# fr34za/multilinear

Measured on NVIDIA B200. Metric: pcs_commit_melem_per_s, higher is better.
Workload: dtype u128

## Files before the change

include/multilinear_b200_instr.h:

```cpp
#ifndef MULTILINEAR_B200_INSTR_H
#define MULTILINEAR_B200_INSTR_H
#include <stddef.h>
#include <stdint.h>

#ifdef __cplusplus
extern "C" {
#endif

void ml_trace_dump(void);

int ml_profile_enable(int on);
int ml_profile_reset(void);
int ml_profile_get(int id, double *total_ms, uint64_t *launches, double *alg_bytes);
int ml_profile_get_max(int id, double *mean_ms, uint64_t *launches, double *alg_bytes);
int ml_microbench(const char *what, size_t n, int iters, double *ms_out, double *work_out);

struct ml_shard;
int ml_shard_phase_ms(const struct ml_shard *sh, double *out, int cap);
struct ml_pcs_shard;
int ml_pcs_shard_phase_ms(const struct ml_pcs_shard *sh, double *out, int cap);
struct ml_bpcs_shard;
int ml_bpcs_shard_phase_ms(const struct ml_bpcs_shard *sh, double *out, int cap);

#ifdef __cplusplus
}
#endif
#endif
```

multilinear_b200/api.py:

```python
import ctypes as C

import numpy as np

from ._lib import MlError, NotPowerOfTwo, NotRsCode, SizeMismatch, check, load

M = 340282366920938463463374557953744961537
LOG_BLOWUP = 1
NUM_QUERIES = 128
_sz = C.c_size_t


def _p(a):
    return C.c_void_p(a.ctypes.data)


def aligned_empty(nbytes, align=64):
    raw = np.empty(nbytes + align, dtype=np.uint8)
    off = (-raw.ctypes.data) % align
    return raw[off:off + nbytes]


def elems_empty(n):
    return aligned_empty(16 * n).reshape(n, 16)

# ... 1028 lines not shown
    def free(self):
        if self.h is not None and self.h.value:
            load().ml_wsumcheck_shard_free(self.h)
        self.h = None

    def __del__(self):
        try:
            self.free()
        except Exception:
            pass


_INSTR = None


def microbench(what, n, iters):
    global _INSTR
    if _INSTR is None:
        import os
        load()
        _INSTR = C.CDLL(os.path.join(os.path.dirname(os.path.abspath(__file__)), "libmlb_instr.so"))
    ms, work = C.c_double(0), C.c_double(0)
    check(_INSTR.ml_microbench(what.encode(), _sz(n), C.c_int(iters), C.byref(ms), C.byref(work)))
    return ms.value, work.value
```

multilinear_b200/csrc/field.cuh:

```cuda
#pragma once
#include <cstdint>
#include <cuda_runtime.h>

namespace mlb {

struct fe {
    uint32_t v[4];
};

#define MLB_C0 0xFFFFFFFFu
#define MLB_C1 0x00002CFFu
#define MLB_M0 0x00000001u
#define MLB_M1 0xFFFFD300u
#define MLB_M2 0xFFFFFFFFu
#define MLB_M3 0xFFFFFFFFu

__device__ __forceinline__ fe fe_zero() { return fe{{0u, 0u, 0u, 0u}}; }
__device__ __forceinline__ fe fe_one() { return fe{{1u, 0u, 0u, 0u}}; }
__device__ __forceinline__ fe fe_from_u4(uint4 x) { return fe{{x.x, x.y, x.z, x.w}}; }
__device__ __forceinline__ uint4 fe_to_u4(fe a) { return make_uint4(a.v[0], a.v[1], a.v[2], a.v[3]); }
__device__ __forceinline__ fe fe_load(const fe* p) { return fe_from_u4(*reinterpret_cast<const uint4*>(p)); }
__device__ __forceinline__ fe fe_load_nc(const fe* p) { return fe_from_u4(__ldg(reinterpret_cast<const uint4*>(p))); }
__device__ __forceinline__ void fe_store(fe* p, fe a) { *reinterpret_cast<uint4*>(p) = fe_to_u4(a); }
__device__ __forceinline__ bool fe_eq(fe a, fe b) {
// ... 83 lines not shown
    uint32_t y0 = x0, y1 = x1, y2 = x2, y3 = x3, k1, q0, q1, q2, k2;
    asm("mad.lo.cc.u32 %0, %5, %7, %0; madc.hi.cc.u32 %1, %5, %7, %1; madc.lo.cc.u32 %2, %6, %8, %2; madc.hi.cc.u32 %3, %6, %8, %3; addc.u32 %4, 0, 0;"
        : "+r"(y0), "+r"(y1), "+r"(y2), "+r"(y3), "=&r"(k1) : "r"(x4), "r"(x5), "r"(c0), "r"(c1));
    asm("mul.lo.u32 %0, %3, %5; mul.hi.u32 %1, %3, %5; mad.lo.cc.u32 %0, %4, %6, %0; madc.hi.cc.u32 %1, %4, %6, %1; addc.u32 %2, 0, 0;"
        : "=&r"(q0), "=&r"(q1), "=&r"(q2) : "r"(x4), "r"(x5), "r"(c1), "r"(c0));
    asm("add.cc.u32 %0, %0, %4; addc.cc.u32 %1, %1, %5; addc.cc.u32 %2, %2, %6; addc.u32 %3, 0, 0;"
        : "+r"(y1), "+r"(y2), "+r"(y3), "=&r"(k2) : "r"(q0), "r"(q1), "r"(q2));
    uint32_t m = 0u - (k1 + k2);
    asm("add.cc.u32 %0, %0, %4; addc.cc.u32 %1, %1, %5; addc.cc.u32 %2, %2, 0; addc.u32 %3, %3, 0;"
        : "+r"(y0), "+r"(y1), "+r"(y2), "+r"(y3) : "r"(m & c0), "r"(m & c1));
    return fe_new(fe{{y0, y1, y2, y3}});
}


#define MLB_K45 11520u
__device__ __forceinline__ fe fe_reduce_wide_v2(const uint32_t p[8]) {
    uint32_t a1 = p[1], a2 = p[2], a3 = p[3], a4, a5, x0, x1, x2, x3, x4, x5;
    const uint32_t k = MLB_K45;
    asm("mad.lo.cc.u32 %0, %4, %6, %0; madc.hi.cc.u32 %1, %4, %6, %1; madc.lo.cc.u32 %2, %5, %6, %2; madc.hi.u32 %3, %5, %6, 0;"
        : "+r"(a1), "+r"(a2), "+r"(a3), "=&r"(a4) : "r"(p[4]), "r"(p[6]), "r"(k));
    asm("mad.lo.cc.u32 %0, %4, %6, %0; madc.hi.cc.u32 %1, %4, %6, %1; madc.lo.cc.u32 %2, %5, %6, %2; madc.hi.u32 %3, %5, %6, 0;"
        : "+r"(a2), "+r"(a3), "+r"(a4), "=&r"(a5) : "r"(p[5]), "r"(p[7]), "r"(k));
    asm("sub.cc.u32 %0, %6, %12; subc.cc.u32 %1, %7, %13; subc.cc.u32 %2, %8, %14; subc.cc.u32 %3, %9, %15; subc.cc.u32 %4, %10, 0; subc.u32 %5, %11, 0;"
        : "=&r"(x0), "=&r"(x1), "=&r"(x2), "=&r"(x3), "=&r"(x4), "=&r"(x5)
        : "r"(p[0]), "r"(a1), "r"(a2), "r"(a3), "r"(a4), "r"(a5), "r"(p[4]), "r"(p[5]), "r"(p[6]), "r"(p[7]));
    const unsigned long long U = (unsigned long long)x4 * MLB_K45 + ((unsigned long long)(x5 * MLB_K45) << 32);
    uint32_t b1, b2, b3, k1, y0, y1, y2, y3, k2;
    asm("add.cc.u32 %0, %4, %7; addc.cc.u32 %1, %5, %8; addc.cc.u32 %2, %6, 0; addc.u32 %3, 0, 0;"
        : "=&r"(b1), "=&r"(b2), "=&r"(b3), "=&r"(k1) : "r"(x1), "r"(x2), "r"(x3), "r"((uint32_t)U), "r"((uint32_t)(U >> 32)));
    asm("sub.cc.u32 %0, %5, %9; subc.cc.u32 %1, %6, %10; subc.cc.u32 %2, %7, 0; subc.cc.u32 %3, %8, 0; subc.u32 %4, 0, 0;"
        : "=&r"(y0), "=&r"(y1), "=&r"(y2), "=&r"(y3), "=&r"(k2) : "r"(x0), "r"(b1), "r"(b2), "r"(b3), "r"(x4), "r"(x5));
    uint32_t z0, z1, z2, z3, g;
    asm("add.cc.u32 %0, %5, %9; addc.cc.u32 %1, %6, %10; addc.cc.u32 %2, %7, 0; addc.cc.u32 %3, %8, 0; addc.u32 %4, %11, %12;"
        : "=&r"(z0), "=&r"(z1), "=&r"(z2), "=&r"(z3), "=&r"(g)
        : "r"(y0), "r"(y1), "r"(y2), "r"(y3), "r"(MLB_C0), "r"(MLB_C1), "r"(k1), "r"(k2));
    return fe{{g ? z0 : y0, g ? z1 : y1, g ? z2 : y2, g ? z3 : y3}};
}
#ifndef MLB_REDUCE_V
#define MLB_REDUCE_V 2
#endif
template <int V>
__device__ __forceinline__ fe fe_reduce_wide_t(const uint32_t p[8]) { return V == 1 ? fe_reduce_wide_v1(p) : fe_reduce_wide_v2(p); }
__device__ __forceinline__ fe fe_reduce_wide(const uint32_t p[8]) { return fe_reduce_wide_t<MLB_REDUCE_V>(p); }
template <int V>
__device__ __forceinline__ fe fe_mul_t(const fe& a, const fe& b) {
    uint32_t p[8];
    fe_mul_wide(p, a, b);
    return fe_reduce_wide_t<V>(p);
}

__device__ __forceinline__ fe fe_mul(const fe& a, const fe& b) {
    uint32_t p[8];
    fe_mul_wide(p, a, b);
    return fe_reduce_wide(p);
}
__device__ __forceinline__ fe fe_sqr(const fe& a) { return fe_mul(a, a); }

__device__ inline fe fe_pow_u64(fe base, unsigned long long e) {
    fe r = fe_one();
    while (e) {
        if (e & 1ull) r = fe_mul(r, base);
        base = fe_sqr(base);
        e >>= 1;
    }
    return r;
}

struct fe_acc {
    uint32_t w[9];
};
__device__ __forceinline__ void acc_zero(fe_acc& s) {
#pragma unroll
// ... 23 lines not shown
```

multilinear_b200/csrc/internal.h:

```cpp
#pragma once
#include <atomic>
#include <cstdarg>
#include <cstdint>
#include <cstdio>
#include <cstring>
#include <map>
#include <mutex>
#include <vector>

#include <cuda_runtime.h>

#include "../../include/multilinear_b200.h"
#include "../../include/multilinear_b200_instr.h"

namespace mlb {

void set_error(const char* fmt, ...);
extern std::atomic<unsigned long long> g_kernel_launches;
#define MLB_COUNT_LAUNCH() (++::mlb::g_kernel_launches)

#define MLB_CUDA(expr)                                                                          \
    do {                                                                                        \
        cudaError_t _e = (expr);                                                                \
        if (_e != cudaSuccess) {                                                                \
// ... 60 lines not shown
    while (e) { if (e & 1) r = hfe_mul(r, b); b = hfe_mul(b, b); e >>= 1; }
    return r;
}
static inline hfe hfe_inv(hfe a) { return a ? hfe_pow(a, HFE_M - 2) : 0; }
static inline hfe hfe_div(hfe a, hfe b) { return hfe_mul(a, hfe_inv(b)); }
static inline hfe hfe_half(hfe a) { return hfe_mul(a, (HFE_M + 1) >> 1); }
static inline bool hfe_pow2_generator(uint64_t log_size, hfe* out) {
    if (log_size > 40) return false;
    *out = hfe_pow(3, (HFE_M - 1) >> log_size);
    return true;
}
static inline bool is_pow2(size_t n) { return n && !(n & (n - 1)); }
static inline unsigned ilog2(size_t n) { return 63u - (unsigned)__builtin_clzll((unsigned long long)n); }

struct fe;

static const int LO_BITS = 12;
struct RootTables {
    int log_n = 0;
    fe* lo = nullptr;
    fe* hi = nullptr;
    fe* lo_ninv = nullptr;
    hfe gen = 0;
    fe* pass_tw[2][4] = {{nullptr, nullptr, nullptr, nullptr}, {nullptr, nullptr, nullptr, nullptr}};
};
struct Ctx {
    int device = -1;
    cudaStream_t stream = nullptr;
    std::map<int, RootTables> roots;
    std::mutex roots_mu;
    fe* small_fwd = nullptr;
    fe* small_inv = nullptr;
    int sm_count = 148;
};
int get_ctx(Ctx** out);
cudaStream_t lib_stream(Ctx* ctx);
int lib_stream_create(cudaStream_t* out, bool non_blocking);
int lib_stream_destroy(cudaStream_t s);
int get_root_tables(Ctx* ctx, int log_n, cudaStream_t s, const RootTables** out);

int dev_alloc_async(void** p, size_t bytes, cudaStream_t s);
int dev_free_async(void* p, cudaStream_t s);

int ntt_launch(Ctx* ctx, const fe* in, fe* out, int log_n, bool inverse, bool rs_zero_padded, cudaStream_t s, bool bitrev_in = false);
static inline bool ntt_fuses_bitrev(int log_n) { return log_n > 12; }
int powers_launch(Ctx* ctx, int log_n, fe* out, cudaStream_t s);
int bit_reverse_launch(const void* in, void* out, size_t n, size_t elem_bytes, cudaStream_t s);
// ... 81 lines not shown
```

multilinear_b200/csrc/microbench.cu:

```cuda
#include "field.cuh"
#include "internal.h"
#include "sha256.cuh"
#include <cstdlib>
#include <string>

namespace mlb {

template <int MODE, int V = MLB_REDUCE_V>
__global__ void __launch_bounds__(256) mb_field_kernel(fe* out, int iters, fe seed) {
    const unsigned tid = blockIdx.x * blockDim.x + threadIdx.x;
    fe a[4], w = seed;
    w.v[0] ^= tid;
#pragma unroll
    for (int i = 0; i < 4; i++) { a[i] = seed; a[i].v[1] ^= tid * 4 + i; a[i] = fe_new(a[i]); }
    w = fe_new(w);
    for (int it = 0; it < iters; it++) {
#pragma unroll
        for (int i = 0; i < 4; i += (MODE == 0 ? 1 : 2)) {
            if (MODE == 0) a[i] = fe_mul_t<V>(a[i], w);
            else {
                fe v = fe_mul_t<V>(a[i + 1], w), u = a[i];
                a[i] = fe_add(u, v);
                a[i + 1] = fe_sub(u, v);
            }
        }
    }
    fe r = fe_add(fe_add(a[0], a[1]), fe_add(a[2], a[3]));
    if (r.v[0] == 0x12345678u && r.v[3] == 0x9abcdef0u) fe_store(out + tid, r);
}
template <int MODE, int FMA_ADD, int ROT = 0, int MINB = 1>
__global__ void __launch_bounds__(128, MINB) mb_sha_kernel(uint32_t* out, int iters, uint32_t seed) {
    const unsigned tid = blockIdx.x * blockDim.x + threadIdx.x;
    uint32_t h[8], g[8];
#pragma unroll
    for (int i = 0; i < 8; i++) { h[i] = seed + tid * 8 + i; g[i] = seed ^ (tid + i); }
    for (int it = 0; it < iters; it++) {
// ... 30 lines not shown
            if (MODE == 0 || MODE == 5) asm volatile("add.u32 %0, %0, %1;" : "+r"(a[i]) : "r"(b[i]));
            if (MODE == 1 || MODE == 5 || MODE == 6 || MODE == 9) asm volatile("mad.lo.u32 %0, %0, %1, %2;" : "+r"(b[i]) : "r"(m), "r"(a[i]));
            if (MODE == 12 || MODE == 13 || MODE == 14) asm volatile("fma.rn.f64 %0, %0, %1, %2;" : "+d"(fd[i]) : "d"(fm), "d"(fa));
            if (MODE == 14) asm volatile("shf.r.wrap.b32 %0, %0, %0, 7;" : "+r"(a[i]));
            if (MODE == 2 || MODE == 7 || MODE == 13) asm volatile("{\n\t.reg .u32 lo;\n\tcvt.u32.u64 lo, %0;\n\tmad.wide.u32 %0, lo, %1, %0;\n\t}" : "+l"(wd[i]) : "r"(m));
            if (MODE == 10 || MODE == 11) asm volatile("mul.hi.u32 %0, %0, %1;" : "+r"(b[i]) : "r"(m));
            if (MODE == 11) asm volatile("shf.r.wrap.b32 %0, %0, %0, 7;" : "+r"(a[i]));
            if (MODE == 3 || MODE == 6 || MODE == 7 || MODE == 8 || MODE == 9) asm volatile("shf.r.wrap.b32 %0, %0, %0, 7;" : "+r"(a[i]));
            if (MODE == 4 || MODE == 8 || MODE == 9) asm volatile("lop3.b32 %0, %0, %1, %2, 0x96;" : "+r"(b[i]) : "r"(a[i]), "r"(m));
        }
    }
    uint32_t r = 0;
#pragma unroll
    for (int i = 0; i < 8; i++) r += a[i] + b[i] + (uint32_t)wd[i] + (uint32_t)(wd[i] >> 32) + (uint32_t)__double2uint_rz(fd[i]);
    if (r == 0x12345678u) out[tid] = r;
}

__global__ void __launch_bounds__(256) mb_copy_kernel(const uint4* __restrict__ in, uint4* __restrict__ out, size_t n) {
    size_t i = (size_t)blockIdx.x * blockDim.x + threadIdx.x;
    const size_t stride = (size_t)gridDim.x * blockDim.x;
    for (; i < n; i += stride) out[i] = __ldg(in + i);
}

}

using namespace mlb;

extern "C" int ml_microbench(const char* what, size_t n, int iters, double* ms_out, double* work_out) {
    Ctx* ctx;
    MLB_TRY(get_ctx(&ctx));
// ... 4 lines not shown
    void* buf = nullptr;
    const std::string w(what);
    size_t bytes = w == "copy" ? 2 * n : (n + 1024) * 16;
    MLB_CUDA(cudaMalloc(&buf, bytes));
    MLB_CUDA(cudaMemsetAsync(buf, 1, bytes, s));
    fe seed = fe{{0x9e3779b9u, 0x7f4a7c15u, 0xbf58476du, 0x14057b7eu}};
    double best = 1e30;
    for (int rep = 0; rep < 6; rep++) {
        MLB_CUDA(cudaEventRecord(e0, s));
        if (w == "modmul") mb_field_kernel<0><<<(unsigned)((n + 255) / 256), 256, 0, s>>>((fe*)buf, iters, seed);
        else if (w == "butterfly") mb_field_kernel<1><<<(unsigned)((n + 255) / 256), 256, 0, s>>>((fe*)buf, iters, seed);
        else if (w == "modmul_v1") mb_field_kernel<0, 1><<<(unsigned)((n + 255) / 256), 256, 0, s>>>((fe*)buf, iters, seed);
        else if (w == "modmul_v2") mb_field_kernel<0, 2><<<(unsigned)((n + 255) / 256), 256, 0, s>>>((fe*)buf, iters, seed);
        else if (w == "butterfly_v1") mb_field_kernel<1, 1><<<(unsigned)((n + 255) / 256), 256, 0, s>>>((fe*)buf, iters, seed);
        else if (w == "butterfly_v2") mb_field_kernel<1, 2><<<(unsigned)((n + 255) / 256), 256, 0, s>>>((fe*)buf, iters, seed);
        else if (w == "sha_leaf") mb_sha_kernel<0, MLB_SHA_ADD_MASK><<<(unsigned)((n + 127) / 128), 128, 0, s>>>((uint32_t*)buf, iters, 0x1234567u);
        else if (w == "sha_node") mb_sha_kernel<1, MLB_SHA_ADD_MASK><<<(unsigned)((n + 127) / 128), 128, 0, s>>>((uint32_t*)buf, iters, 0x1234567u);
#define MB_SHA_VARIANT(M)                                                                                                              \
        else if (w == "sha_leaf_m" #M) mb_sha_kernel<0, M><<<(unsigned)((n + 127) / 128), 128, 0, s>>>((uint32_t*)buf, iters, 0x1234567u); \
        else if (w == "sha_node_m" #M) mb_sha_kernel<1, M><<<(unsigned)((n + 127) / 128), 128, 0, s>>>((uint32_t*)buf, iters, 0x1234567u);
#define MB_SHA_ROT(M, R)                                                                                                               \
        else if (w == "sha_leaf_m" #M "_r" #R) mb_sha_kernel<0, M, R><<<(unsigned)((n + 127) / 128), 128, 0, s>>>((uint32_t*)buf, iters, 0x1234567u); \
        else if (w == "sha_node_m" #M "_r" #R) mb_sha_kernel<1, M, R><<<(unsigned)((n + 127) / 128), 128, 0, s>>>((uint32_t*)buf, iters, 0x1234567u);
        MB_SHA_ROT(2, 1) MB_SHA_ROT(2, 11) MB_SHA_ROT(2, 111) MB_SHA_ROT(2, 101) MB_SHA_ROT(2, 21) MB_SHA_ROT(2, 121) MB_SHA_ROT(2, 211)
        MB_SHA_ROT(0, 1) MB_SHA_ROT(0, 11) MB_SHA_ROT(0, 111) MB_SHA_ROT(0, 121) MB_SHA_ROT(2, 221) MB_SHA_ROT(0, 211)
        MB_SHA_VARIANT(0) MB_SHA_VARIANT(63) MB_SHA_VARIANT(3) MB_SHA_VARIANT(1) MB_SHA_VARIANT(2) MB_SHA_VARIANT(19) MB_SHA_VARIANT(11)
        MB_SHA_VARIANT(27) MB_SHA_VARIANT(59) MB_SHA_VARIANT(43)
        else if (w.rfind("pipe", 0) == 0) {
            const int mode = atoi(what + 4);
            const unsigned gb = (unsigned)((n + 255) / 256);
// ... 27 lines not shown
    cudaFree(buf);
    cudaEventDestroy(e0);
    cudaEventDestroy(e1);
    *ms_out = best;
    if (w.rfind("modmul", 0) == 0) *work_out = (double)n * iters * 4;
    else if (w.rfind("butterfly", 0) == 0) *work_out = (double)n * iters * 2;
    else if (w == "copy") *work_out = 2.0 * (double)n;
    else if (w.rfind("pipe", 0) == 0) {
        const int mode = atoi(what + 4);
        const int per = (mode <= 4 || mode == 10 || mode == 12) ? 1 : (mode == 9 ? 3 : 2);
        *work_out = (double)n * iters * 8 * per;
    }
    else *work_out = (double)n * iters;
    return ML_OK;
}
```

multilinear_b200/csrc/ntt.cu:

```cuda
#include <cstdlib>
#include "field.cuh"
#include "internal.h"

namespace mlb {

static const int NTT_THREADS = 256;
static const int TILE_LOG = 12;

struct PassArgs {
    const fe* in;
    fe* out;
    const fe* small;
    const fe* lo;
    const fe* hi;
    const fe* wtab;
    fe scale;
    int log_n, log_r, log_t, log_a, log_b;
    int last, inverse, zero_padded, scaled_lo, has_scale;
    int bitrev_in;
    int n_passes;
    int radix_log[4];
};

template <int NS, bool LAST>
__device__ __forceinline__ void dif_round(fe* data, const fe* tw, int pitch, int log_r, int log_t, int q, int tid) {
    const int log_lr = LAST ? 0 : log_r - q - NS;
    const int items = 1 << (log_r + log_t - NS);
    for (int w = tid; w < items; w += NTT_THREADS) {
        const int t = w & ((1 << log_t) - 1);
        const int rest = w >> log_t;
        const int l = LAST ? 0 : (rest & ((1 << log_lr) - 1));
        const int blk = rest >> log_lr;
        const int m0 = (blk << (log_r - q)) + l;
        fe x[1 << NS];
#pragma unroll
        for (int j = 0; j < (1 << NS); j++) x[j] = data[(m0 + (j << log_lr)) * pitch + t];
#pragma unroll
        for (int u = 0; u < NS; u++) {
            const int span = 1 << (NS - 1 - u);
#pragma unroll
            for (int j = 0; j < (1 << NS); j++) {
                if (j & span) continue;
                fe a = x[j], b = x[j + span];
                x[j] = fe_add(a, b);
                fe d = fe_sub(a, b);
                if (LAST) {
                    if ((j & (span - 1)) != 0) d = fe_mul(d, tw[(j & (span - 1)) << (q + u)]);
                } else {
                    const int e = (((j & (span - 1)) << log_lr) + l) << (q + u);
                    d = fe_mul(d, tw[e]);
                }
                x[j + span] = d;
            }
        }
#pragma unroll
        for (int j = 0; j < (1 << NS); j++) data[(m0 + (j << log_lr)) * pitch + t] = x[j];
    }
}

__global__ void __launch_bounds__(NTT_THREADS, 3) ntt_pass_kernel(PassArgs p) {
    extern __shared__ uint4 smem_raw[];
    fe* data = reinterpret_cast<fe*>(smem_raw);
    const int R = 1 << p.log_r, T = 1 << p.log_t;
    const int pitch = (p.last && T > 1) ? T + 1 : T;
    fe* tw = data + (size_t)R * pitch;
    const int tid = threadIdx.x;
    const size_t tile = blockIdx.x;

    for (int i = tid; i < (R >> 1); i += NTT_THREADS) tw[i] = fe_load_nc(p.small + ((size_t)i << (12 - p.log_r)));
    if (tid == 0 && R == 1) tw[0] = fe_one();

    size_t a = 0, bt = 0, ap = 0, k0_base = 0;
    const int log_rb = p.log_r + p.log_b;
    if (!p.last) {
        const int log_tiles_b = p.log_b - p.log_t;
        bt = tile & (((size_t)1 << log_tiles_b) - 1);
        a = tile >> log_tiles_b;
    } else if (p.n_passes > 1) {
        const int log_k0_tiles = p.radix_log[0] - p.log_t;
        k0_base = (tile & (((size_t)1 << log_k0_tiles) - 1)) << p.log_t;
        ap = tile >> log_k0_tiles;
    }
    const int log_a_rest = p.log_a - (p.n_passes > 1 ? p.radix_log[0] : 0);

    const int tile_elems = R * T;
// ... 38 lines not shown
        else if (ns == 2) { if (last) dif_round<2, true>(data, tw, pitch, p.log_r, p.log_t, q, tid); else dif_round<2, false>(data, tw, pitch, p.log_r, p.log_t, q, tid); }
        else { if (last) dif_round<1, true>(data, tw, pitch, p.log_r, p.log_t, q, tid); else dif_round<1, false>(data, tw, pitch, p.log_r, p.log_t, q, tid); }
        q += ns;
        __syncthreads();
    }

    if (!p.last) {
        const size_t base = (a << log_rb) + (bt << p.log_t);
        const size_t nmask = ((size_t)1 << p.log_n) - 1;
#pragma unroll 4
        for (int idx = tid; idx < tile_elems; idx += NTT_THREADS) {
            const int t = idx & (T - 1), pos = idx >> p.log_t;
            const size_t k = __brev((unsigned)pos) >> (32 - p.log_r);
            const size_t b = (bt << p.log_t) + t;
            fe v = data[pos * pitch + t];
            if (p.wtab) {
                v = fe_mul(v, fe_load_nc(p.wtab + (k << p.log_b) + b));
            } else {
                size_t e = (k * b) << p.log_a;
                if (p.inverse) e = (((size_t)1 << p.log_n) - e) & nmask;
                if (e != 0 || p.scaled_lo) {
                    fe w = fe_load_nc(p.lo + (e & (((size_t)1 << LO_BITS) - 1)));
                    if (e >> LO_BITS) w = fe_mul(w, fe_load_nc(p.hi + (e >> LO_BITS)));
                    v = fe_mul(v, w);
                }
            }
            fe_store(p.out + base + (k << p.log_b) + t, v);
        }
    } else {
        size_t mid = 0;
        {
// ... 14 lines not shown
            if (p.has_scale) v = fe_mul(v, p.scale);
            fe_store(p.out + (k0_base + t) + (mid << log_r0) + (k << p.log_a), v);
        }
    }
}

__global__ void root_tables_kernel(fe* lo, fe* hi, fe* lo_ninv, fe gen, fe gen_hi, fe ninv, unsigned n_lo, unsigned n_hi) {
    unsigned i = blockIdx.x * blockDim.x + threadIdx.x;
    if (i < n_lo) {
        fe w = fe_pow_u64(gen, i);
        fe_store(lo + i, w);
        fe_store(lo_ninv + i, fe_mul(w, ninv));
    }
    if (i < n_hi) fe_store(hi + i, fe_pow_u64(gen_hi, i));
}
__global__ void small_roots_kernel(fe* fwd, fe* inv, fe w, fe winv) {
    unsigned i = blockIdx.x * blockDim.x + threadIdx.x;
    if (i < 2048) {
        fe_store(fwd + i, fe_pow_u64(w, i));
        fe_store(inv + i, fe_pow_u64(winv, i));
    }
}
__global__ void pass_table_kernel(fe* out, const fe* lo, const fe* hi, int log_n, int log_a, int log_b, int inverse, size_t count) {
    size_t i = (size_t)blockIdx.x * blockDim.x + threadIdx.x;
    const size_t stride = (size_t)gridDim.x * blockDim.x;
    const size_t nmask = ((size_t)1 << log_n) - 1;
    for (; i < count; i += stride) {
        const size_t k = i >> log_b, b = i & (((size_t)1 << log_b) - 1);
        size_t e = (k * b) << log_a;
        if (inverse) e = (((size_t)1 << log_n) - e) & nmask;
        fe w = fe_load_nc(lo + (e & (((size_t)1 << LO_BITS) - 1)));
        if (e >> LO_BITS) w = fe_mul(w, fe_load_nc(hi + (e >> LO_BITS)));
        fe_store(out + i, w);
    }
}

__global__ void powers_kernel(fe* out, const fe* lo, const fe* hi, size_t n) {
    size_t i = (size_t)blockIdx.x * blockDim.x + threadIdx.x;
    const size_t stride = (size_t)gridDim.x * blockDim.x;
    for (; i < n; i += stride) {
        fe w = fe_load_nc(lo + (i & (((size_t)1 << LO_BITS) - 1)));
        if (i >> LO_BITS) w = fe_mul(w, fe_load_nc(hi + (i >> LO_BITS)));
        fe_store(out + i, w);
    }
}

static fe to_dev_fe(hfe x) {
    fe r;
    r.v[0] = (uint32_t)x; r.v[1] = (uint32_t)(x >> 32); r.v[2] = (uint32_t)(x >> 64); r.v[3] = (uint32_t)(x >> 96);
    return r;
}

int get_root_tables(Ctx* ctx, int log_n, cudaStream_t s, const RootTables** out) {
    std::lock_guard<std::mutex> lock(ctx->roots_mu);
    if (!ctx->small_fwd) {
        hfe w;
        hfe_pow2_generator(12, &w);
        MLB_CUDA(cudaMalloc((void**)&ctx->small_fwd, 2048 * 16));
        MLB_CUDA(cudaMalloc((void**)&ctx->small_inv, 2048 * 16));
        small_roots_kernel<<<8, 256, 0, s>>>(ctx->small_fwd, ctx->small_inv, to_dev_fe(w), to_dev_fe(hfe_inv(w)));
        MLB_KERNEL_CHECK();
        MLB_CUDA(cudaStreamSynchronize(s));
    }
    auto it = ctx->roots.find(log_n);
    if (it == ctx->roots.end()) {
        RootTables rt;
        rt.log_n = log_n;
        if (!hfe_pow2_generator((uint64_t)log_n, &rt.gen)) { set_error("no 2^%d-th root of unity", log_n); return ML_ERR_OUT_OF_RANGE; }
        const size_t n = (size_t)1 << log_n;
        const unsigned n_lo = (unsigned)(n < ((size_t)1 << LO_BITS) ? n : ((size_t)1 << LO_BITS));
        const unsigned n_hi = (unsigned)(n >> LO_BITS ? n >> LO_BITS : 1);
        if (cudaMalloc((void**)&rt.lo, (size_t)n_lo * 16) != cudaSuccess || cudaMalloc((void**)&rt.lo_ninv, (size_t)n_lo * 16) != cudaSuccess ||
            cudaMalloc((void**)&rt.hi, (size_t)n_hi * 16) != cudaSuccess) {
            cudaGetLastError();
// ... 1 lines not shown
            set_error("root tables for 2^%d: device allocation failed", log_n);
            return ML_ERR_ALLOC;
        }
        hfe gen_hi = hfe_pow(rt.gen, (hfe)1 << LO_BITS);
        hfe ninv = hfe_inv(hfe_new((hfe)n));
        unsigned m = n_lo > n_hi ? n_lo : n_hi;
        root_tables_kernel<<<(m + 255) / 256, 256, 0, s>>>(rt.lo, rt.hi, rt.lo_ninv, to_dev_fe(rt.gen), to_dev_fe(gen_hi), to_dev_fe(ninv), n_lo, n_hi);
        MLB_KERNEL_CHECK();
        MLB_CUDA(cudaStreamSynchronize(s));
        it = ctx->roots.emplace(log_n, rt).first;
    }
    *out = &it->second;
    return ML_OK;
}

static int get_pass_table(Ctx* ctx, int log_n, bool inverse, int pass, int log_a, int log_r, int log_b, cudaStream_t s, const fe** out) {
    *out = nullptr;
    const size_t count = (size_t)1 << (log_r + log_b);
    if (count * 16 > ((size_t)1 << 30)) return ML_OK;
    static const bool no_wtab = getenv("MLB_NTT_NO_WTAB") != nullptr;
    if (no_wtab) return ML_OK;
    std::lock_guard<std::mutex> lock(ctx->roots_mu);
    RootTables& rt = ctx->roots[log_n];
    fe*& slot = rt.pass_tw[inverse ? 1 : 0][pass];
    if (!slot) {
        fe* tab;
        if (cudaMalloc((void**)&tab, count * 16) != cudaSuccess) { cudaGetLastError(); return ML_OK; }
        size_t blocks = (count + 255) / 256;
        if (blocks > (size_t)ctx->sm_count * 16) blocks = (size_t)ctx->sm_count * 16;
        const fe* lo = (inverse && pass == 0) ? rt.lo_ninv : rt.lo;
        pass_table_kernel<<<(unsigned)blocks, 256, 0, s>>>(tab, lo, rt.hi, log_n, log_a, log_b, inverse ? 1 : 0, count);
        MLB_KERNEL_CHECK();
        MLB_CUDA(cudaStreamSynchronize(s));
        slot = tab;
    }
    *out = slot;
    return ML_OK;
}

int powers_launch(Ctx* ctx, int log_n, fe* out, cudaStream_t s) {
    const RootTables* rt;
    MLB_TRY(get_root_tables(ctx, log_n, s, &rt));
    const size_t n = (size_t)1 << log_n;
    size_t blocks = (n + 255) / 256;
    if (blocks > (size_t)ctx->sm_count * 16) blocks = (size_t)ctx->sm_count * 16;
    powers_kernel<<<(unsigned)blocks, 256, 0, s>>>(out, rt->lo, rt->hi, n);
    MLB_KERNEL_CHECK();
    return ML_OK;
}

int ntt_launch(Ctx* ctx, const fe* in, fe* out, int log_n, bool inverse, bool rs_zero_padded, cudaStream_t s, bool bitrev_in) {
    if (bitrev_in && !(rs_zero_padded && !inverse && log_n > TILE_LOG)) { set_error("ntt: bit-reversed input needs a multi-pass RS encode"); return ML_ERR_ARG; }
    MLB_CUDA(cudaFuncSetAttribute(ntt_pass_kernel, cudaFuncAttributeMaxDynamicSharedMemorySize, 112 * 1024));
    const RootTables* rt;
    MLB_TRY(get_root_tables(ctx, log_n, s, &rt));
    if (log_n == 0) {
        if (in != out) MLB_CUDA(cudaMemcpyAsync(out, in, 16, cudaMemcpyDeviceToDevice, s));
        return ML_OK;
    }
    int n_passes = log_n <= TILE_LOG ? 1 : (log_n + 8) / 9;
    int radix_log[4] = {0, 0, 0, 0};
    if (n_passes > 4) { set_error("NTT size 2^%d not supported", log_n); return ML_ERR_ARG; }
    for (int p = 0; p < n_passes; p++) radix_log[p] = log_n / n_passes + (p < log_n % n_passes ? 1 : 0);

    struct TmpGuard {
        fe* p = nullptr;
        cudaStream_t s;
        explicit TmpGuard(cudaStream_t st) : s(st) {}
// ... 14 lines not shown
    for (int p = 0; p < 4; p++) a.radix_log[p] = radix_log[p];
    int log_a = 0;
    for (int p = 0; p < n_passes; p++) {
        a.last = p == n_passes - 1;
        a.in = p == 0 ? in : tmp;
        a.out = a.last ? out : tmp;
        a.log_r = radix_log[p];
        a.log_a = log_a;
        a.log_b = log_n - log_a - a.log_r;
        a.log_t = n_passes == 1 ? 0 : TILE_LOG - a.log_r;
        a.zero_padded = (rs_zero_padded && p == 0) ? 1 : 0;
        a.bitrev_in = (bitrev_in && p == 0) ? 1 : 0;
        a.scaled_lo = (inverse && p == 0 && n_passes > 1) ? 1 : 0;
        a.lo = a.scaled_lo ? rt->lo_ninv : rt->lo;
        a.wtab = nullptr;
        if (!a.last) MLB_TRY(get_pass_table(ctx, log_n, inverse, p, a.log_a, a.log_r, a.log_b, s, &a.wtab));
        a.has_scale = (inverse && n_passes == 1) ? 1 : 0;
        if (a.has_scale) a.scale = to_dev_fe(hfe_inv(hfe_new((hfe)1 << log_n)));
        const int R = 1 << a.log_r, T = 1 << a.log_t;
        const int pitch = (a.last && T > 1) ? T + 1 : T;
        const size_t smem = ((size_t)R * pitch + (R >> 1) + 1) * 16;
        const size_t tiles = ((size_t)1 << log_n) >> (a.log_r + a.log_t);
        ntt_pass_kernel<<<(unsigned)tiles, NTT_THREADS, smem, s>>>(a);
        MLB_KERNEL_CHECK();
        log_a += a.log_r;
    }
    return ML_OK;
}

__global__ void bit_reverse_kernel(const uint4* in, uint4* out, size_t n, int bits) {
    size_t i = (size_t)blockIdx.x * blockDim.x + threadIdx.x;
    const size_t stride = (size_t)gridDim.x * blockDim.x;
    for (; i < n; i += stride) {
        size_t j = (bits && (i >> bits) == 0) ? (size_t)(__brevll((unsigned long long)i) >> (64 - bits)) : i;
        out[i] = in[j];
    }
// ... 15 lines not shown
```

Baseline: 1884.

## Precompute shifted twiddle limbs for constant multiplication in NTT passes

Adds a constant-multiplier form (fe4c) that stores each twiddle together with its products by 2^32, 2^64 and 2^96 reduced mod p, so a multiply by a known twiddle becomes a 4x4 limb accumulation followed by a small fold instead of a full 8-limb wide reduction. The in-kernel small-root table, shared-memory twiddle cache and later-pass twiddle tables now use this form, and a test entry point plus microbenchmarks are added. The cost is four times the twiddle memory and shared-memory footprint, which raises the dynamic smem cap and may reduce occupancy, plus extra global table traffic for passes after the first.

```diff
diff --git a/include/multilinear_b200_instr.h b/include/multilinear_b200_instr.h
--- a/include/multilinear_b200_instr.h
+++ b/include/multilinear_b200_instr.h
@@ -14,6 +14,7 @@
 int ml_profile_get(int id, double *total_ms, uint64_t *launches, double *alg_bytes);
 int ml_profile_get_max(int id, double *mean_ms, uint64_t *launches, double *alg_bytes);
 int ml_microbench(const char *what, size_t n, int iters, double *ms_out, double *work_out);
+int ml_const_mul(const uint8_t *a, const uint8_t *b, size_t n, uint8_t *out);
 
 struct ml_shard;
 int ml_shard_phase_ms(const struct ml_shard *sh, double *out, int cap);
diff --git a/multilinear_b200/api.py b/multilinear_b200/api.py
--- a/multilinear_b200/api.py
+++ b/multilinear_b200/api.py
@@ -1066,12 +1066,28 @@
 _INSTR = None
 
 
-def microbench(what, n, iters):
+def microbench_lib():
     global _INSTR
     if _INSTR is None:
         import os
         load()
         _INSTR = C.CDLL(os.path.join(os.path.dirname(os.path.abspath(__file__)), "libmlb_instr.so"))
+    return _INSTR
+
+
+def microbench(what, n, iters):
+    lib = microbench_lib()
     ms, work = C.c_double(0), C.c_double(0)
-    check(_INSTR.ml_microbench(what.encode(), _sz(n), C.c_int(iters), C.byref(ms), C.byref(work)))
+    check(lib.ml_microbench(what.encode(), _sz(n), C.c_int(iters), C.byref(ms), C.byref(work)))
     return ms.value, work.value
+
+
+def const_mul(a, b):
+    lib = microbench_lib()
+    n = len(a)
+    ab = b"".join(int(x).to_bytes(16, "little") for x in a)
+    bb = b"".join(int(x).to_bytes(16, "little") for x in b)
+    out = (C.c_uint8 * (16 * n))()
+    check(lib.ml_const_mul(ab, bb, _sz(n), out))
+    raw = bytes(out)
+    return [int.from_bytes(raw[16 * i:16 * i + 16], "little") for i in range(n)]
diff --git a/multilinear_b200/csrc/field.cuh b/multilinear_b200/csrc/field.cuh
--- a/multilinear_b200/csrc/field.cuh
+++ b/multilinear_b200/csrc/field.cuh
@@ -121,16 +121,7 @@
 
 
 #define MLB_K45 11520u
-__device__ __forceinline__ fe fe_reduce_wide_v2(const uint32_t p[8]) {
-    uint32_t a1 = p[1], a2 = p[2], a3 = p[3], a4, a5, x0, x1, x2, x3, x4, x5;
-    const uint32_t k = MLB_K45;
-    asm("mad.lo.cc.u32 %0, %4, %6, %0; madc.hi.cc.u32 %1, %4, %6, %1; madc.lo.cc.u32 %2, %5, %6, %2; madc.hi.u32 %3, %5, %6, 0;"
-        : "+r"(a1), "+r"(a2), "+r"(a3), "=&r"(a4) : "r"(p[4]), "r"(p[6]), "r"(k));
-    asm("mad.lo.cc.u32 %0, %4, %6, %0; madc.hi.cc.u32 %1, %4, %6, %1; madc.lo.cc.u32 %2, %5, %6, %2; madc.hi.u32 %3, %5, %6, 0;"
-        : "+r"(a2), "+r"(a3), "+r"(a4), "=&r"(a5) : "r"(p[5]), "r"(p[7]), "r"(k));
-    asm("sub.cc.u32 %0, %6, %12; subc.cc.u32 %1, %7, %13; subc.cc.u32 %2, %8, %14; subc.cc.u32 %3, %9, %15; subc.cc.u32 %4, %10, 0; subc.u32 %5, %11, 0;"
-        : "=&r"(x0), "=&r"(x1), "=&r"(x2), "=&r"(x3), "=&r"(x4), "=&r"(x5)
-        : "r"(p[0]), "r"(a1), "r"(a2), "r"(a3), "r"(a4), "r"(a5), "r"(p[4]), "r"(p[5]), "r"(p[6]), "r"(p[7]));
+__device__ __forceinline__ fe fe_fold_small(uint32_t x0, uint32_t x1, uint32_t x2, uint32_t x3, uint32_t x4, uint32_t x5) {
     const unsigned long long U = (unsigned long long)x4 * MLB_K45 + ((unsigned long long)(x5 * MLB_K45) << 32);
     uint32_t b1, b2, b3, k1, y0, y1, y2, y3, k2;
     asm("add.cc.u32 %0, %4, %7; addc.cc.u32 %1, %5, %8; addc.cc.u32 %2, %6, 0; addc.u32 %3, 0, 0;"
@@ -143,6 +134,19 @@
         : "r"(y0), "r"(y1), "r"(y2), "r"(y3), "r"(MLB_C0), "r"(MLB_C1), "r"(k1), "r"(k2));
     return fe{{g ? z0 : y0, g ? z1 : y1, g ? z2 : y2, g ? z3 : y3}};
 }
+
+__device__ __forceinline__ fe fe_reduce_wide_v2(const uint32_t p[8]) {
+    uint32_t a1 = p[1], a2 = p[2], a3 = p[3], a4, a5, x0, x1, x2, x3, x4, x5;
+    const uint32_t k = MLB_K45;
+    asm("mad.lo.cc.u32 %0, %4, %6, %0; madc.hi.cc.u32 %1, %4, %6, %1; madc.lo.cc.u32 %2, %5, %6, %2; madc.hi.u32 %3, %5, %6, 0;"
+        : "+r"(a1), "+r"(a2), "+r"(a3), "=&r"(a4) : "r"(p[4]), "r"(p[6]), "r"(k));
+    asm("mad.lo.cc.u32 %0, %4, %6, %0; madc.hi.cc.u32 %1, %4, %6, %1; madc.lo.cc.u32 %2, %5, %6, %2; madc.hi.u32 %3, %5, %6, 0;"
+        : "+r"(a2), "+r"(a3), "+r"(a4), "=&r"(a5) : "r"(p[5]), "r"(p[7]), "r"(k));
+    asm("sub.cc.u32 %0, %6, %12; subc.cc.u32 %1, %7, %13; subc.cc.u32 %2, %8, %14; subc.cc.u32 %3, %9, %15; subc.cc.u32 %4, %10, 0; subc.u32 %5, %11, 0;"
+        : "=&r"(x0), "=&r"(x1), "=&r"(x2), "=&r"(x3), "=&r"(x4), "=&r"(x5)
+        : "r"(p[0]), "r"(a1), "r"(a2), "r"(a3), "r"(a4), "r"(a5), "r"(p[4]), "r"(p[5]), "r"(p[6]), "r"(p[7]));
+    return fe_fold_small(x0, x1, x2, x3, x4, x5);
+}
 #ifndef MLB_REDUCE_V
 #define MLB_REDUCE_V 2
 #endif
@@ -163,6 +167,55 @@
 }
 __device__ __forceinline__ fe fe_sqr(const fe& a) { return fe_mul(a, a); }
 
+struct fe4c {
+    fe b[4];
+};
+__device__ __forceinline__ fe fe_mul_c4(const fe& a, const fe4c& c) {
+    uint32_t e0, e1, e2, e3, e4 = 0u, o1, o2, o3, o4, o5 = 0u;
+    asm("mul.lo.u32 %0, %4, %5; mul.hi.u32 %1, %4, %5; mul.lo.u32 %2, %4, %6; mul.hi.u32 %3, %4, %6;"
+        : "=&r"(e0), "=&r"(e1), "=&r"(e2), "=&r"(e3) : "r"(a.v[0]), "r"(c.b[0].v[0]), "r"(c.b[0].v[2]));
+    asm("mul.lo.u32 %0, %4, %5; mul.hi.u32 %1, %4, %5; mul.lo.u32 %2, %4, %6; mul.hi.u32 %3, %4, %6;"
+        : "=&r"(o1), "=&r"(o2), "=&r"(o3), "=&r"(o4) : "r"(a.v[0]), "r"(c.b[0].v[1]), "r"(c.b[0].v[3]));
+#pragma unroll
+    for (int i = 1; i < 4; i++) {
+        asm("mad.lo.cc.u32 %0, %5, %6, %0; madc.hi.cc.u32 %1, %5, %6, %1; madc.lo.cc.u32 %2, %5, %7, %2; madc.hi.cc.u32 %3, %5, %7, %3; addc.u32 %4, %4, 0;"
+            : "+r"(e0), "+r"(e1), "+r"(e2), "+r"(e3), "+r"(e4) : "r"(a.v[i]), "r"(c.b[i].v[0]), "r"(c.b[i].v[2]));
+        asm("mad.lo.cc.u32 %0, %5, %6, %0; madc.hi.cc.u32 %1, %5, %6, %1; madc.lo.cc.u32 %2, %5, %7, %2; madc.hi.cc.u32 %3, %5, %7, %3; addc.u32 %4, %4, 0;"
+            : "+r"(o1), "+r"(o2), "+r"(o3), "+r"(o4), "+r"(o5) : "r"(a.v[i]), "r"(c.b[i].v[1]), "r"(c.b[i].v[3]));
+    }
+    uint32_t s1, s2, s3, s4, s5;
+    asm("add.cc.u32 %0, %5, %9; addc.cc.u32 %1, %6, %10; addc.cc.u32 %2, %7, %11; addc.cc.u32 %3, %8, %12; addc.u32 %4, %13, 0;"
+        : "=&r"(s1), "=&r"(s2), "=&r"(s3), "=&r"(s4), "=&r"(s5)
+        : "r"(e1), "r"(e2), "r"(e3), "r"(e4), "r"(o1), "r"(o2), "r"(o3), "r"(o4), "r"(o5));
+    return fe_fold_small(e0, s1, s2, s3, s4, s5);
+}
+__device__ __forceinline__ fe4c fe4c_make(const fe& b) {
+    fe4c c;
+    c.b[0] = b;
+#pragma unroll
+    for (int i = 1; i < 4; i++) {
+        const uint32_t p[8] = {0u, c.b[i - 1].v[0], c.b[i - 1].v[1], c.b[i - 1].v[2], c.b[i - 1].v[3], 0u, 0u, 0u};
+        c.b[i] = fe_reduce_wide(p);
+    }
+    return c;
+}
+__device__ __forceinline__ fe4c fe4c_load(const fe4c* p) {
+    fe4c c;
+#pragma unroll
+    for (int i = 0; i < 4; i++) c.b[i] = fe_load(&p->b[i]);
+    return c;
+}
+__device__ __forceinline__ fe4c fe4c_load_nc(const fe4c* p) {
+    fe4c c;
+#pragma unroll
+    for (int i = 0; i < 4; i++) c.b[i] = fe_load_nc(&p->b[i]);
+    return c;
+}
+__device__ __forceinline__ void fe4c_store(fe4c* p, const fe4c& c) {
+#pragma unroll
+    for (int i = 0; i < 4; i++) fe_store(&p->b[i], c.b[i]);
+}
+
 __device__ inline fe fe_pow_u64(fe base, unsigned long long e) {
     fe r = fe_one();
     while (e) {
diff --git a/multilinear_b200/csrc/internal.h b/multilinear_b200/csrc/internal.h
--- a/multilinear_b200/csrc/internal.h
+++ b/multilinear_b200/csrc/internal.h
@@ -98,6 +98,7 @@
 static inline unsigned ilog2(size_t n) { return 63u - (unsigned)__builtin_clzll((unsigned long long)n); }
 
 struct fe;
+struct fe4c;
 
 static const int LO_BITS = 12;
 struct RootTables {
@@ -106,15 +107,15 @@
     fe* hi = nullptr;
     fe* lo_ninv = nullptr;
     hfe gen = 0;
-    fe* pass_tw[2][4] = {{nullptr, nullptr, nullptr, nullptr}, {nullptr, nullptr, nullptr, nullptr}};
+    void* pass_tw[2][4] = {{nullptr, nullptr, nullptr, nullptr}, {nullptr, nullptr, nullptr, nullptr}};
 };
 struct Ctx {
     int device = -1;
     cudaStream_t stream = nullptr;
     std::map<int, RootTables> roots;
     std::mutex roots_mu;
-    fe* small_fwd = nullptr;
-    fe* small_inv = nullptr;
+    fe4c* small_fwd = nullptr;
+    fe4c* small_inv = nullptr;
     int sm_count = 148;
 };
 int get_ctx(Ctx** out);
diff --git a/multilinear_b200/csrc/microbench.cu b/multilinear_b200/csrc/microbench.cu
--- a/multilinear_b200/csrc/microbench.cu
+++ b/multilinear_b200/csrc/microbench.cu
@@ -6,7 +6,7 @@
 
 namespace mlb {
 
-template <int MODE, int V = MLB_REDUCE_V>
+template <int MODE, int V = MLB_REDUCE_V, bool C4 = false>
 __global__ void __launch_bounds__(256) mb_field_kernel(fe* out, int iters, fe seed) {
     const unsigned tid = blockIdx.x * blockDim.x + threadIdx.x;
     fe a[4], w = seed;
@@ -14,12 +14,13 @@
 #pragma unroll
     for (int i = 0; i < 4; i++) { a[i] = seed; a[i].v[1] ^= tid * 4 + i; a[i] = fe_new(a[i]); }
     w = fe_new(w);
+    const fe4c w4 = fe4c_make(w);
     for (int it = 0; it < iters; it++) {
 #pragma unroll
         for (int i = 0; i < 4; i += (MODE == 0 ? 1 : 2)) {
-            if (MODE == 0) a[i] = fe_mul_t<V>(a[i], w);
+            if (MODE == 0) a[i] = C4 ? fe_mul_c4(a[i], w4) : fe_mul_t<V>(a[i], w);
             else {
-                fe v = fe_mul_t<V>(a[i + 1], w), u = a[i];
+                fe v = C4 ? fe_mul_c4(a[i + 1], w4) : fe_mul_t<V>(a[i + 1], w), u = a[i];
                 a[i] = fe_add(u, v);
                 a[i + 1] = fe_sub(u, v);
             }
@@ -80,6 +81,12 @@
 #pragma unroll
     for (int i = 0; i < 8; i++) r += a[i] + b[i] + (uint32_t)wd[i] + (uint32_t)(wd[i] >> 32) + (uint32_t)__double2uint_rz(fd[i]);
     if (r == 0x12345678u) out[tid] = r;
+}
+
+__global__ void __launch_bounds__(256) const_mul_kernel(const fe* __restrict__ a, const fe* __restrict__ b, fe* __restrict__ out, size_t n) {
+    size_t i = (size_t)blockIdx.x * blockDim.x + threadIdx.x;
+    const size_t stride = (size_t)gridDim.x * blockDim.x;
+    for (; i < n; i += stride) fe_store(out + i, fe_mul_c4(fe_load(a + i), fe4c_make(fe_load(b + i))));
 }
 
 __global__ void __launch_bounds__(256) mb_copy_kernel(const uint4* __restrict__ in, uint4* __restrict__ out, size_t n) {
@@ -114,6 +121,8 @@
         else if (w == "modmul_v2") mb_field_kernel<0, 2><<<(unsigned)((n + 255) / 256), 256, 0, s>>>((fe*)buf, iters, seed);
         else if (w == "butterfly_v1") mb_field_kernel<1, 1><<<(unsigned)((n + 255) / 256), 256, 0, s>>>((fe*)buf, iters, seed);
         else if (w == "butterfly_v2") mb_field_kernel<1, 2><<<(unsigned)((n + 255) / 256), 256, 0, s>>>((fe*)buf, iters, seed);
+        else if (w == "modmul_c4") mb_field_kernel<0, MLB_REDUCE_V, true><<<(unsigned)((n + 255) / 256), 256, 0, s>>>((fe*)buf, iters, seed);
+        else if (w == "butterfly_c4") mb_field_kernel<1, MLB_REDUCE_V, true><<<(unsigned)((n + 255) / 256), 256, 0, s>>>((fe*)buf, iters, seed);
         else if (w == "sha_leaf") mb_sha_kernel<0, MLB_SHA_ADD_MASK><<<(unsigned)((n + 127) / 128), 128, 0, s>>>((uint32_t*)buf, iters, 0x1234567u);
         else if (w == "sha_node") mb_sha_kernel<1, MLB_SHA_ADD_MASK><<<(unsigned)((n + 127) / 128), 128, 0, s>>>((uint32_t*)buf, iters, 0x1234567u);
 #define MB_SHA_VARIANT(M)                                                                                                              \
@@ -171,3 +180,30 @@
     else *work_out = (double)n * iters;
     return ML_OK;
 }
+
+extern "C" int ml_const_mul(const uint8_t* a, const uint8_t* b, size_t n, uint8_t* out) {
+    Ctx* ctx;
+    MLB_TRY(get_ctx(&ctx));
+    cudaStream_t s = ctx->stream;
+    if (n == 0) return ML_OK;
+    fe* buf = nullptr;
+    MLB_CUDA(cudaMalloc((void**)&buf, 3 * n * 16));
+    int st = ML_OK;
+    if (cudaMemcpyAsync(buf, a, n * 16, cudaMemcpyHostToDevice, s) != cudaSuccess ||
+        cudaMemcpyAsync(buf + n, b, n * 16, cudaMemcpyHostToDevice, s) != cudaSuccess) {
+        set_error("ml_const_mul: copy to device failed");
+        st = ML_ERR_CUDA;
+    }
+    if (st == ML_OK) {
+        size_t blocks = (n + 255) / 256;
+        if (blocks > (size_t)ctx->sm_count * 16) blocks = (size_t)ctx->sm_count * 16;
+        const_mul_kernel<<<(unsigned)blocks, 256, 0, s>>>(buf, buf + n, buf + 2 * n, n);
+        if (cudaGetLastError() != cudaSuccess || cudaMemcpyAsync(out, buf + 2 * n, n * 16, cudaMemcpyDeviceToHost, s) != cudaSuccess ||
+            cudaStreamSynchronize(s) != cudaSuccess) {
+            set_error("ml_const_mul: kernel or copy failed");
+            st = ML_ERR_CUDA;
+        }
+    }
+    cudaFree(buf);
+    return st;
+}
diff --git a/multilinear_b200/csrc/ntt.cu b/multilinear_b200/csrc/ntt.cu
--- a/multilinear_b200/csrc/ntt.cu
+++ b/multilinear_b200/csrc/ntt.cu
@@ -6,14 +6,16 @@
 
 static const int NTT_THREADS = 256;
 static const int TILE_LOG = 12;
+static const int NTT_MIN_CTAS = 3;
 
 struct PassArgs {
     const fe* in;
     fe* out;
-    const fe* small;
+    const fe4c* small;
     const fe* lo;
     const fe* hi;
     const fe* wtab;
+    const fe4c* wtab4;
     fe scale;
     int log_n, log_r, log_t, log_a, log_b;
     int last, inverse, zero_padded, scaled_lo, has_scale;
@@ -23,7 +25,7 @@
 };
 
 template <int NS, bool LAST>
-__device__ __forceinline__ void dif_round(fe* data, const fe* tw, int pitch, int log_r, int log_t, int q, int tid) {
+__device__ __forceinline__ void dif_round(fe* data, const fe4c* tw, int pitch, int log_r, int log_t, int q, int tid) {
     const int log_lr = LAST ? 0 : log_r - q - NS;
     const int items = 1 << (log_r + log_t - NS);
     for (int w = tid; w < items; w += NTT_THREADS) {
@@ -45,10 +47,10 @@
                 x[j] = fe_add(a, b);
                 fe d = fe_sub(a, b);
                 if (LAST) {
-                    if ((j & (span - 1)) != 0) d = fe_mul(d, tw[(j & (span - 1)) << (q + u)]);
+                    if ((j & (span - 1)) != 0) d = fe_mul_c4(d, fe4c_load(tw + ((j & (span - 1)) << (q + u))));
                 } else {
                     const int e = (((j & (span - 1)) << log_lr) + l) << (q + u);
-                    d = fe_mul(d, tw[e]);
+                    d = fe_mul_c4(d, fe4c_load(tw + e));
                 }
                 x[j + span] = d;
             }
@@ -58,17 +60,16 @@
     }
 }
 
-__global__ void __launch_bounds__(NTT_THREADS, 3) ntt_pass_kernel(PassArgs p) {
+__global__ void __launch_bounds__(NTT_THREADS, NTT_MIN_CTAS) ntt_pass_kernel(PassArgs p) {
     extern __shared__ uint4 smem_raw[];
     fe* data = reinterpret_cast<fe*>(smem_raw);
     const int R = 1 << p.log_r, T = 1 << p.log_t;
     const int pitch = (p.last && T > 1) ? T + 1 : T;
-    fe* tw = data + (size_t)R * pitch;
+    fe4c* tw = reinterpret_cast<fe4c*>(data + (size_t)R * pitch);
     const int tid = threadIdx.x;
     const size_t tile = blockIdx.x;
 
-    for (int i = tid; i < (R >> 1); i += NTT_THREADS) tw[i] = fe_load_nc(p.small + ((size_t)i << (12 - p.log_r)));
-    if (tid == 0 && R == 1) tw[0] = fe_one();
+    for (int i = tid; i < (R >> 1); i += NTT_THREADS) fe4c_store(tw + i, fe4c_load_nc(p.small + ((size_t)i << (12 - p.log_r))));
 
     size_t a = 0, bt = 0, ap = 0, k0_base = 0;
     const int log_rb = p.log_r + p.log_b;
@@ -137,7 +138,9 @@
             const size_t k = __brev((unsigned)pos) >> (32 - p.log_r);
             const size_t b = (bt << p.log_t) + t;
             fe v = data[pos * pitch + t];
-            if (p.wtab) {
+            if (p.wtab4) {
+                v = fe_mul_c4(v, fe4c_load_nc(p.wtab4 + (k << p.log_b) + b));
+            } else if (p.wtab) {
                 v = fe_mul(v, fe_load_nc(p.wtab + (k << p.log_b) + b));
             } else {
                 size_t e = (k * b) << p.log_a;
@@ -182,14 +185,17 @@
     }
     if (i < n_hi) fe_store(hi + i, fe_pow_u64(gen_hi, i));
 }
-__global__ void small_roots_kernel(fe* fwd, fe* inv, fe w, fe winv) {
+__global__ void small_roots_kernel(fe4c* fwd, fe4c* inv, fe w, fe winv) {
     unsigned i = blockIdx.x * blockDim.x + threadIdx.x;
     if (i < 2048) {
-        fe_store(fwd + i, fe_pow_u64(w, i));
-        fe_store(inv + i, fe_pow_u64(winv, i));
-    }
-}
-__global__ void pass_table_kernel(fe* out, const fe* lo, const fe* hi, int log_n, int log_a, int log_b, int inverse, size_t count) {
+        fe4c_store(fwd + i, fe4c_make(fe_pow_u64(w, i)));
+        fe4c_store(inv + i, fe4c_make(fe_pow_u64(winv, i)));
+    }
+}
+__device__ __forceinline__ void tw_store(fe* p, const fe& w) { fe_store(p, w); }
+__device__ __forceinline__ void tw_store(fe4c* p, const fe& w) { fe4c_store(p, fe4c_make(w)); }
+template <typename T>
+__global__ void pass_table_kernel(T* out, const fe* lo, const fe* hi, int log_n, int log_a, int log_b, int inverse, size_t count) {
     size_t i = (size_t)blockIdx.x * blockDim.x + threadIdx.x;
     const size_t stride = (size_t)gridDim.x * blockDim.x;
     const size_t nmask = ((size_t)1 << log_n) - 1;
@@ -199,7 +205,7 @@
         if (inverse) e = (((size_t)1 << log_n) - e) & nmask;
         fe w = fe_load_nc(lo + (e & (((size_t)1 << LO_BITS) - 1)));
         if (e >> LO_BITS) w = fe_mul(w, fe_load_nc(hi + (e >> LO_BITS)));
-        fe_store(out + i, w);
+        tw_store(out + i, w);
     }
 }
 
@@ -224,8 +230,8 @@
     if (!ctx->small_fwd) {
         hfe w;
         hfe_pow2_generator(12, &w);
-        MLB_CUDA(cudaMalloc((void**)&ctx->small_fwd, 2048 * 16));
-        MLB_CUDA(cudaMalloc((void**)&ctx->small_inv, 2048 * 16));
+        MLB_CUDA(cudaMalloc((void**)&ctx->small_fwd, 2048 * sizeof(fe4c)));
+        MLB_CUDA(cudaMalloc((void**)&ctx->small_inv, 2048 * sizeof(fe4c)));
         small_roots_kernel<<<8, 256, 0, s>>>(ctx->small_fwd, ctx->small_inv, to_dev_fe(w), to_dev_fe(hfe_inv(w)));
         MLB_KERNEL_CHECK();
         MLB_CUDA(cudaStreamSynchronize(s));
@@ -257,27 +263,33 @@
     return ML_OK;
 }
 
-static int get_pass_table(Ctx* ctx, int log_n, bool inverse, int pass, int log_a, int log_r, int log_b, cudaStream_t s, const fe** out) {
+static int get_pass_table(Ctx* ctx, int log_n, bool inverse, int pass, int log_a, int log_r, int log_b, cudaStream_t s, const fe** out,
+                          const fe4c** out4) {
     *out = nullptr;
+    *out4 = nullptr;
     const size_t count = (size_t)1 << (log_r + log_b);
-    if (count * 16 > ((size_t)1 << 30)) return ML_OK;
+    const bool c4 = pass > 0;
+    const size_t bytes = count * (c4 ? sizeof(fe4c) : sizeof(fe));
+    if (bytes > ((size_t)1 << 30)) return ML_OK;
     static const bool no_wtab = getenv("MLB_NTT_NO_WTAB") != nullptr;
     if (no_wtab) return ML_OK;
     std::lock_guard<std::mutex> lock(ctx->roots_mu);
     RootTables& rt = ctx->roots[log_n];
-    fe*& slot = rt.pass_tw[inverse ? 1 : 0][pass];
+    void*& slot = rt.pass_tw[inverse ? 1 : 0][pass];
     if (!slot) {
-        fe* tab;
-        if (cudaMalloc((void**)&tab, count * 16) != cudaSuccess) { cudaGetLastError(); return ML_OK; }
+        void* tab;
+        if (cudaMalloc(&tab, bytes) != cudaSuccess) { cudaGetLastError(); return ML_OK; }
         size_t blocks = (count + 255) / 256;
         if (blocks > (size_t)ctx->sm_count * 16) blocks = (size_t)ctx->sm_count * 16;
         const fe* lo = (inverse && pass == 0) ? rt.lo_ninv : rt.lo;
-        pass_table_kernel<<<(unsigned)blocks, 256, 0, s>>>(tab, lo, rt.hi, log_n, log_a, log_b, inverse ? 1 : 0, count);
+        if (c4) pass_table_kernel<<<(unsigned)blocks, 256, 0, s>>>((fe4c*)tab, lo, rt.hi, log_n, log_a, log_b, inverse ? 1 : 0, count);
+        else pass_table_kernel<<<(unsigned)blocks, 256, 0, s>>>((fe*)tab, lo, rt.hi, log_n, log_a, log_b, inverse ? 1 : 0, count);
         MLB_KERNEL_CHECK();
         MLB_CUDA(cudaStreamSynchronize(s));
         slot = tab;
     }
-    *out = slot;
+    if (c4) *out4 = (const fe4c*)slot;
+    else *out = (const fe*)slot;
     return ML_OK;
 }
 
@@ -294,7 +306,7 @@
 
 int ntt_launch(Ctx* ctx, const fe* in, fe* out, int log_n, bool inverse, bool rs_zero_padded, cudaStream_t s, bool bitrev_in) {
     if (bitrev_in && !(rs_zero_padded && !inverse && log_n > TILE_LOG)) { set_error("ntt: bit-reversed input needs a multi-pass RS encode"); return ML_ERR_ARG; }
-    MLB_CUDA(cudaFuncSetAttribute(ntt_pass_kernel, cudaFuncAttributeMaxDynamicSharedMemorySize, 112 * 1024));
+    MLB_CUDA(cudaFuncSetAttribute(ntt_pass_kernel, cudaFuncAttributeMaxDynamicSharedMemorySize, 192 * 1024));
     const RootTables* rt;
     MLB_TRY(get_root_tables(ctx, log_n, s, &rt));
     if (log_n == 0) {
@@ -339,12 +351,13 @@
         a.scaled_lo = (inverse && p == 0 && n_passes > 1) ? 1 : 0;
         a.lo = a.scaled_lo ? rt->lo_ninv : rt->lo;
         a.wtab = nullptr;
-        if (!a.last) MLB_TRY(get_pass_table(ctx, log_n, inverse, p, a.log_a, a.log_r, a.log_b, s, &a.wtab));
+        a.wtab4 = nullptr;
+        if (!a.last) MLB_TRY(get_pass_table(ctx, log_n, inverse, p, a.log_a, a.log_r, a.log_b, s, &a.wtab, &a.wtab4));
         a.has_scale = (inverse && n_passes == 1) ? 1 : 0;
         if (a.has_scale) a.scale = to_dev_fe(hfe_inv(hfe_new((hfe)1 << log_n)));
         const int R = 1 << a.log_r, T = 1 << a.log_t;
         const int pitch = (a.last && T > 1) ? T + 1 : T;
-        const size_t smem = ((size_t)R * pitch + (R >> 1) + 1) * 16;
+        const size_t smem = (size_t)R * pitch * sizeof(fe) + (size_t)(R >> 1) * sizeof(fe4c);
         const size_t tiles = ((size_t)1 << log_n) >> (a.log_r + a.log_t);
         ntt_pass_kernel<<<(unsigned)tiles, NTT_THREADS, smem, s>>>(a);
         MLB_KERNEL_CHECK();
```

After: 1901 (median of 6 runs). Within noise of the previous version (+0.9%).
